# JingInAI/Quantize

Hardware: AMD Instinct MI355X
Metric: quant-conv2d images/sec at batch 256 (ResNet-50, W8A8) (higher is better)
Workload: dtype int8

## Files before the change

### quantize_amd/csrc/qe_conv_plan.hip

```cpp
#include "qe_conv_plan.hpp"

#include <algorithm>
#include <cstdlib>

namespace qe {

static int knob(const char *name, int dflt)
{
    const char *e = env_get(name);
    return e ? atoi(e) : dflt;
}

static size_t align_up(size_t v, size_t a) { return (v + a - 1) / a * a; }

static const int kNiw[3][3] = {{7, 4, 2}, {4, 2, 1}, {2, 1, 0}};
static const int kWN[3] = {1, 2, 4};

struct PlanFront {
    MfmaPlan p;
    int max_tiles = 0;
    bool ok = false;
};

static PlanFront plan_front(const qe_conv_shape *sh)
// ... 227 lines not shown
    if (p.family == MfmaFamily::None) p = plan_flat_s2(f, sh, w_bits);
    if (p.family == MfmaFamily::None) p = plan_flatg(f, sh, w_bits);
    if (p.family == MfmaFamily::None) {
        if (stem_shape(sh)) p = plan_stem(f, sh);
        else {
            p = plan_sm2(f, sh);
            if (p.family == MfmaFamily::None) p = plan_halo(f, sh);
        }
    }
    if (p.family == MfmaFamily::None) return f.p;
    return plan_tables(p, sh);
}

static qe_conv_shape dense_shape(const qe_conv_shape *sh)
{
    qe_conv_shape d = *sh;
    d.H = (sh->H - 1) / sh->stride + 1;
    d.W = (sh->W - 1) / sh->stride + 1;
    d.stride = 1;
    return d;
}

static MfmaPlan make_plan(const qe_conv_shape *sh, int x_bits, int w_bits)
{
    const bool expand = x_bits < 8;
    const int sub_env = knob("QE_SUBSAMPLE", -1);
    const int p_out = ((sh->H - 1) / std::max(1, (int)sh->stride) + 1) * ((sh->W - 1) / std::max(1, (int)sh->stride) + 1);
    const bool sub_x4 = x_bits == 4 && sh->stride == 2 && (sh->W % 2) == 0 && ((int64_t)sh->H * sh->W % 2) == 0 &&
                        knob("QE_SUB_X4", 1) != 0;
    const bool sub = sh->KH == 1 && sh->KW == 1 && sh->stride > 1 && sh->padding == 0 && sub_env != 0 &&
                     (sub_env > 0 || p_out <= 256 || sub_x4);
    const qe_conv_shape ds = dense_shape(sh);
    if (x_bits == 4 && !sub && knob("QE_X4", 1) != 0) {
        const PlanFront f = plan_front(sh);
        MfmaPlan q = f.ok ? plan_flat(f, sh, w_bits, true) : f.p;
        if (q.family == MfmaFamily::FlatX4) {
            q = plan_tables(q, sh);
            q.prep_total = q.total;
            return q;
        }
    }
    MfmaPlan p = make_plan8(sub ? &ds : sh, w_bits);
    p.prep_total = p.total;
    if (p.family != MfmaFamily::None && sub) {
        p.sub = true;
        p.sub_x4 = sub_x4;
        p.sub_off = align_up(p.total, 256);
        p.total = p.sub_off + align_up((size_t)ds.N * ds.IC * ds.H * ds.W, 256);
    } else if (sub) {
        p = make_plan8(sh, w_bits);
        p.prep_total = p.total;
    }
    if (p.family != MfmaFamily::None && expand) {
        p.expand = true;
        p.xe_off = align_up(p.total, 256);
        p.total = p.xe_off + align_up((size_t)sh->N * sh->IC * sh->H * sh->W, 256);
    }
    return p;
}

MfmaPlan plan_prepared(const qe_conv_shape *sh, int x_bits, int w_bits)
{
    qe_conv_shape s1 = *sh;
    const int64_t img = (int64_t)sh->IC * sh->H * sh->W;
    s1.N = img >= 64 ? 1 : (int)((64 + img - 1) / img);
    return make_plan(&s1, x_bits, w_bits);
}

uint64_t prepared_layout(const MfmaPlan &p, const qe_conv_shape *sh)
{
    if (p.family == MfmaFamily::None || p.prep_total == 0) return 0;
    uint64_t h = 1469598103934665603ull;
    auto mix = [&](uint64_t v) { h = (h ^ v) * 1099511628211ull; };
    mix(p.family == MfmaFamily::Stem ? 1 : 0); mix((uint64_t)p.OCP); mix((uint64_t)p.NG); mix((uint64_t)p.KK); mix((uint64_t)sh->KH); mix((uint64_t)sh->KW);
    mix((uint64_t)sh->IC); mix((uint64_t)sh->OC); mix((uint64_t)p.prep_total); mix((uint64_t)p.ep_off); mix((uint64_t)p.ws_off);
    return h | 1ull;
}

struct PwrFit {
    int tw = 0, ks = 0, groups = 1;
    bool s2 = false;
};

static bool pwr_plan(const qe_conv_shape *sh, const qe_qparam *x, const qe_qparam *w, uintptr_t xa, PwrFit *pl)
{
    const int mode = knob("QE_PWR", 2);
    if (mode == 0) return false;
    if (sh->KH != 1 || sh->KW != 1 || sh->padding != 0 || (sh->stride != 1 && sh->stride != 2)) return false;
    if (x->n_bits != 8 || w->n_bits != 8 || x->n_param != 1) return false;
    if (sh->IC != 64 && sh->IC != 128 && sh->IC != 256) return false;
    if (sh->OC % 32 != 0 || sh->OC < 128 || sh->N < 1) return false;
    const bool s2 = sh->stride == 2;
    if (s2 && ((sh->H & 1) || (sh->W & 7) || sh->W > 64 || knob("QE_PWR_S2", 1) == 0)) return false;
    const int OH = s2 ? sh->H / 2 : sh->H, OW = s2 ? sh->W / 2 : sh->W;
    const int64_t P = (int64_t)OH * OW;
    const int tw = (P % 224 == 0) ? 224 : ((P % 196 == 0) ? 196 : 0);
    if (tw == 0) return false;
    if (s2 && (tw % OW != 0 || tw / OW > 8)) return false;
    if (mode == 1 && !s2 && P != tw) return false;
    if ((int64_t)sh->N * sh->IC * sh->H * sh->W < 16 || (int64_t)sh->OC * P >= (1ll << 29) || (int64_t)sh->IC * sh->H * sh->W >= (1ll << 31)) return false;
    if ((reinterpret_cast<uintptr_t>(w->data) & 15) != 0 || (xa & (s2 ? 7 : 3)) != 0) return false;
    if ((reinterpret_cast<uintptr_t>(w->scale) & 3) != 0) return false;
    const int ks = sh->IC / 32;
    const int waves = ks == 8 ? 8 : 4;
    if (sh->OC < 64 * waves) return false;
    const int strips = sh->OC / 32;
    const int g = knob("QE_PWR_GROUPS", 0);
    pl->tw = tw; pl->ks = ks; pl->groups = (g >= 1 && strips % g == 0) ? g : 1; pl->s2 = s2;
    return true;
}

static int pwr7_plan(const qe_conv_shape *sh, const qe_qparam *x, const qe_qparam *w, uintptr_t xa, int *groups)
{
    if (knob("QE_PWR", 2) == 0 || knob("QE_PWR7", 1) == 0) return 0;
    if (sh->KH != 1 || sh->KW != 1 || sh->stride != 1 || sh->padding != 0 || sh->H * sh->W != 49) return 0;
    if (x->n_bits != 8 || w->n_bits != 8 || x->n_param != 1) return 0;
    if (sh->IC != 128 && sh->IC != 256 && sh->IC != 512) return 0;
    const int gi = sh->IC == 512 ? 2 : 4;
    if (sh->OC % 32 != 0 || sh->OC < 512 || sh->N < gi || sh->N % gi != 0) return 0;
    if ((int64_t)sh->N * sh->IC * 49 >= (1ll << 31) || (int64_t)sh->OC * 49 >= (1ll << 29)) return 0;
    if ((reinterpret_cast<uintptr_t>(w->data) & 15) != 0 || (xa & 15) != 0) return 0;
    const int tiles = sh->N / gi, strips = sh->OC / 32;
    int g = 1;
    while (tiles * g < kNumCU && strips % (2 * g) == 0 && strips / (2 * g) >= 8) g *= 2;
    const int ge = knob("QE_PWR_GROUPS", 0);
    *groups = (ge >= 1 && strips % ge == 0) ? ge : g;
    return gi;
}

static bool flatd_plan(const qe_conv_shape *sh, const qe_qparam *x, const qe_qparam *w, uintptr_t xa)
{
    if (sh->KH != 1 || sh->KW != 1 || sh->stride != 1 || sh->padding != 0) return false;
    if (x->n_bits != 8 || w->n_bits != 8 || x->n_param != 1) return false;
    if (sh->IC % FD_CK != 0 || sh->IC < 2 * FD_CK || sh->OC < 1 || sh->N < 1) return false;
    const int64_t P = (int64_t)sh->H * sh->W;
    if ((int64_t)sh->N * sh->IC * P < 16 || (int64_t)sh->OC * P >= (1ll << 29) || (int64_t)sh->IC * P >= (1ll << 31)) return false;
    if ((reinterpret_cast<uintptr_t>(w->data) & 15) != 0) return false;
    return P == 49 && sh->OC % 4 == 0 && (xa & 15) == 0;
}

static bool plan_rq_patch(const MfmaPlan &m, const ConvRequest &r, int split)
{
    if (m.GI != 1 || (m.OH * m.OW) % 4 != 0 || (m.TH * m.OW) % 4 != 0) return false;
    if ((r.rq_out & 3) != 0 || knob("QE_RQ_PATCH", 1) == 0) return false;
    return mfma_instance(m, r.sh->KW, split, true, true) != nullptr;
}

static void plan_mfma_launch(ConvPlan &p, const ConvRequest &r, bool rq)
{
    const MfmaPlan &m = p.m;
    const qe_conv_shape *sh = &p.run;
    p.tiles_h = (m.OH + m.TH - 1) / m.TH;
    p.n_pix_tiles = ((sh->N + m.GI - 1) / m.GI) * p.tiles_h;
    p.n_oc_tiles = m.OCP / m.MT;
    const bool flatg = m.family == MfmaFamily::Flatg;
    const bool flat = mfma_is_flat(m.family);
    if (flatg) {
        p.tiles_h = 1;
        p.n_pix_tiles = (sh->N + m.GI - 1) / m.GI;
    } else if (flat) {
        p.tiles_h = m.IHT;
        p.n_pix_tiles = sh->N * p.tiles_h;
    }
    p.blocks = tile_grid(p.n_pix_tiles, p.tiles_h, p.n_oc_tiles, true, p.chunk);
    auto clipped_lo = [](int pad, int stride, int O) { return std::min(O, (pad + stride - 1) / stride); };
    auto clipped_hi = [](int I, int pad, int K, int stride, int O) {
        const int full_last = (I + pad - K) >= 0 ? (I + pad - K) / stride : -1;
        return std::max(0, std::min(O, O - 1 - full_last));
    };
    p.n_top = clipped_lo(sh->padding, sh->stride, m.OH);
    p.n_bot = clipped_hi(sh->H, sh->padding, sh->KH, sh->stride, m.OH);
    p.n_lft = clipped_lo(sh->padding, sh->stride, m.OW);
    p.n_rgt = clipped_hi(sh->W, sh->padding, sh->KW, sh->stride, m.OW);

    if (flat || flatg) {
        p.lds = m.lds;
        if (rq) {
            p.ptab_off = (int)align_up(m.lds, 16);
            p.lds = p.ptab_off + (flatg ? (size_t)m.GI * m.MT * sh->H * sh->W : (size_t)m.MT * 32 * m.ni);
        }
        return;
    }
    const int units = m.GI * m.IHT * ((sh->W + 3) / 4);
    p.split = units <= 64 ? 4 : (units <= 128 ? 2 : 1);
    p.rq_patch = rq && plan_rq_patch(m, r, p.split);
    const size_t stage_bytes = p.rq_patch ? std::max(m.lds, (size_t)32 * 1024) : m.lds;
    size_t lds_e = stage_bytes;
    const size_t tab = (size_t)m.MT * (sh->KH + 1) * (sh->KW + 1) * sizeof(int);
    const size_t off = align_up(stage_bytes, 16);
    if (off + tab <= (size_t)(m.family == MfmaFamily::Sm2 ? MF_MAX_LDS_SM2 : MF_MAX_LDS)) { p.ptab_off = (int)off; lds_e = off + tab; }
    const int ncls = (1 + p.n_top + p.n_bot) * (1 + p.n_lft + p.n_rgt);
    p.ctab = p.ptab_off != 0 && p.n_top + p.n_bot < m.OH && p.n_lft + p.n_rgt < m.OW && ncls <= (sh->KH + 1) * (sh->KW + 1) &&
             knob("QE_CTAB", 1) != 0;
    p.lds = (m.family == MfmaFamily::Ws && !p.ctab) ? m.lds : lds_e;
}

ConvPlan plan_conv(const ConvRequest &r)
{
    ConvPlan p;
    const qe_conv_shape *sh = r.sh;
    p.OH = (sh->H + 2 * sh->padding - sh->KH) / sh->stride + 1;
    p.OW = (sh->W + 2 * sh->padding - sh->KW) / sh->stride + 1;
    if (p.OH > 0 && p.OW > 0) p.y_bytes = align_up((size_t)sh->N * sh->OC * p.OH * p.OW * sizeof(float), 256);
    p.m = make_plan(sh, r.x->n_bits, r.w->n_bits);
    const MfmaPlan &m = p.m;
    if (r.x->n_param != 1 || m.family == MfmaFamily::None) return p;
    p.run = m.sub ? dense_shape(sh) : *sh;
    const qe_conv_shape *rs = &p.run;

    qe_qparam xr = *r.x;
    uintptr_t xa = reinterpret_cast<uintptr_t>(r.x->data);
    if (m.sub_x4 || m.expand) { xr.n_bits = 8; xr.sign = 1; }
    if (m.sub || m.expand) xa = 0;
    if (m.sub_x4) {
        p.pre = PrePass::SubX4;
        p.pre_blocks = ((int64_t)sh->N * sh->IC * rs->H * ((rs->W + 7) / 8) + 255) / 256;
    } else if (m.sub) {
        const int64_t n_planes = (int64_t)sh->N * sh->IC;
        const int nq = (rs->W + 7) / 8;
        int log_nq = 0;
        while ((1 << log_nq) < nq) ++log_nq;
        const int units2 = rs->H << log_nq;
        if (sh->stride == 2 && (sh->H % 2) == 0 && (1 << log_nq) == nq && 16 * nq <= 2 * sh->W && units2 <= 256 &&
            knob("QE_SUB2", 1) != 0) {
            int log_up = 3;
            while ((1 << log_up) < units2) ++log_up;
            p.pre = PrePass::Sub2;
            p.sub2_log_nq = log_nq;
            p.sub2_log_up = log_up;
            const int ppb = (256 >> log_up) * 4;
            p.pre_blocks = (n_planes + ppb - 1) / ppb;
        } else {
            const bool wide = sh->stride == 2 && (sh->W % 4) == 0 && sh->W >= 16;
            const int units = rs->H * ((rs->W + (wide ? 7 : 3)) / (wide ? 8 : 4));
            const int ppb = units >= 1024 ? 1 : 1024 / units;
            p.pre = wide ? PrePass::SubWide : PrePass::SubNarrow;
            p.pre_blocks = (n_planes + ppb - 1) / ppb;
        }
    }
    if (p.pre_blocks > 0x7fffffffLL) return p;

    PwrFit pf;
    int g7 = 1;
    if (r.residual) {
        if (r.rq_bits != 0 && (r.rq_bits != 8 || r.rq_n_param != 1)) return p;
        if (m.sub || m.expand || rs->stride != 1) return p;
        if (pwr_plan(rs, &xr, r.w, xa, &pf)) p.route = ConvRoute::Pwr;
        else if (rs->IC == 512 && (p.pwr7_gi = pwr7_plan(rs, &xr, r.w, xa, &g7)) != 0) p.route = ConvRoute::Pwr7;
        else return p;
        p.fused = true;
    } else {
        const bool rq = r.rq_bits > 0;
        if (rq) {
            if (r.rq_bits != 8 || r.rq_n_param != 1) return p;
            if (m.family == MfmaFamily::Flatg || mfma_is_flat(m.family)) {
                const size_t patch = m.family == MfmaFamily::Flatg ? (size_t)m.GI * m.MT * rs->H * rs->W : (size_t)m.MT * 32 * m.ni;
                if (align_up(m.lds, 16) + patch > (size_t)MF_MAX_LDS) return p;
            }
            p.fused = true;
        }
        const bool pwr_ok = rq ? (r.rq_out & 15) == 0 && knob("QE_PWR_RQ", 1) != 0 : true;
        const bool fd_ok = flatd_plan(rs, &xr, r.w, xa) && knob("QE_FLATD", 1) != 0 &&
                           (!rq || (rs->OC % 32 == 0 && (r.rq_out & 15) == 0 && knob("QE_FLATD_RQ", 1) != 0));
        if (pwr_ok && pwr_plan(rs, &xr, r.w, xa, &pf)) p.route = ConvRoute::Pwr;
        else if (pwr_ok && (rq || (r.out & 15) == 0) && (p.pwr7_gi = pwr7_plan(rs, &xr, r.w, xa, &g7)) != 0) p.route = ConvRoute::Pwr7;
        else if (fd_ok) p.route = ConvRoute::Flatd;
        else p.route = ConvRoute::Mfma;
    }

    if (p.route == ConvRoute::Pwr) {
        p.pwr_tw = pf.tw; p.pwr_ks = pf.ks; p.pwr_groups = pf.groups; p.pwr_s2 = pf.s2;
        const int64_t P = pf.s2 ? (int64_t)(rs->H / 2) * (rs->W / 2) : (int64_t)rs->H * rs->W;
        p.tiles_h = (int)(P / pf.tw);
        p.n_pix_tiles = rs->N * p.tiles_h;
        p.blocks = tile_grid(p.n_pix_tiles, p.tiles_h, pf.groups, true, p.chunk);
    } else if (p.route == ConvRoute::Pwr7) {
        p.pwr_groups = g7;
        p.tiles_h = 1;
        p.n_pix_tiles = rs->N / p.pwr7_gi;
        p.blocks = tile_grid(p.n_pix_tiles, 1, g7, false, p.chunk);
    } else if (p.route == ConvRoute::Flatd) {
        const char *e8 = env_get("QE_FLATD8");
        p.fd_w8 = e8 ? atoi(e8) != 0 && rs->OC > 128 : rs->OC >= 1024;
        const int MT = p.fd_w8 ? 256 : 128;
        p.n_oc_tiles = (rs->OC + MT - 1) / MT;
        p.tiles_h = 1;
        p.n_pix_tiles = (rs->N + 3) / 4;
        p.blocks = tile_grid(p.n_pix_tiles, p.tiles_h, p.n_oc_tiles, true, p.chunk);
    } else {
        plan_mfma_launch(p, r, p.fused);
    }
    if (p.blocks > 0x7fffffffLL) { p.route = ConvRoute::Generic; p.fused = false; }
    return p;
}

}
```

### quantize_amd/csrc/qe_conv_plan.hpp

```cpp
#pragma once
#include "qe_conv_common.hpp"

namespace qe {

constexpr int FD_CK = 64;

enum class MfmaFamily {
    None,
    Halo,
    Ws,
    Sm2,
    Stem,
    Flat,
    FlatS2,
    FlatX4,
    Flatg
};

inline bool mfma_is_flat(MfmaFamily f) { return f == MfmaFamily::Flat || f == MfmaFamily::FlatS2 || f == MfmaFamily::FlatX4; }

struct MfmaPlan {
    MfmaFamily family = MfmaFamily::None;
    int cfg = 0;
    int MT = 0, OCP = 0, NCH = 0, NG = 0, KK = 0, OH = 0, OW = 0;
    int TH = 0, ni = 0, niw = 0, IHT = 0, IWP = 0, ROWMUL = 1, COLMUL = 1;
    int GI = 1, NS = 1;
    bool wraw = false;
    bool expand = false;
    size_t xe_off = 0;
    bool sub = false;
    bool sub_x4 = false;
    size_t sub_off = 0;
    size_t lds = 0;
    size_t wt_bytes = 0, ep_off = 0, ws_off = 0, total = 0;
    size_t prep_total = 0;
};

enum class ConvRoute { Generic, Pwr, Pwr7, Flatd, Mfma };
enum class PrePass { None, SubX4, Sub2, SubWide, SubNarrow };

struct ConvRequest {
    const qe_conv_shape *sh;
    const qe_qparam *x, *w;
    uintptr_t out = 0;
    uintptr_t rq_out = 0;
    int rq_bits = 0;
    int rq_n_param = 1;
    bool residual = false;
};

struct ConvPlan {
    ConvRoute route = ConvRoute::Generic;
    bool fused = false;
    int OH = 0, OW = 0;
    size_t y_bytes = 0;
    MfmaPlan m;
    qe_conv_shape run{};

    PrePass pre = PrePass::None;
    int64_t pre_blocks = 0;
    int sub2_log_up = 0, sub2_log_nq = 0;

    int64_t blocks = 0;
    int chunk = 1, n_pix_tiles = 0, n_oc_tiles = 0, tiles_h = 0;
    size_t lds = 0;

    int pwr_tw = 0, pwr_ks = 0, pwr_groups = 1, pwr7_gi = 0;
    bool pwr_s2 = false;
    bool fd_w8 = false;
    bool rq_patch = false;
    bool ctab = false;
    int ptab_off = 0;
    int n_top = 0, n_bot = 0, n_lft = 0, n_rgt = 0;
    int split = 1;
};

ConvPlan plan_conv(const ConvRequest &rq);
MfmaPlan plan_prepared(const qe_conv_shape *sh, int x_bits, int w_bits);
uint64_t prepared_layout(const MfmaPlan &p, const qe_conv_shape *sh);

MfmaLaunch mfma_instance(const MfmaPlan &m, int KW, int split, bool rq, bool patch);
inline int mfma_kkt(int KK, int KW) { return KK == 1 ? 1 : ((KK == 9 && KW == 3) ? 9 : 0); }

int launch_conv_mfma(const ConvPlan &p, const qe_qparam *x, const qe_qparam *w, const float *bias, const qe_conv_shape *sh,
                     float *out, void *workspace, size_t workspace_bytes, const void *prepared, size_t prepared_bytes,
                     bool use_prepared, hipStream_t s, const RequantHost *rq, const float *res);
int prepare_conv_tables(const MfmaPlan &p, const qe_qparam *w, const float *bias, const qe_conv_shape *sh, void *prepared,
                        size_t prepared_bytes, hipStream_t s);
int launch_pwr(const ConvPlan &p, const qe_qparam *x, const qe_qparam *w, const float *bias, float *out, hipStream_t s,
               const RequantHost *rq, const float *res);
int launch_flatd(const ConvPlan &p, const qe_qparam *x, const qe_qparam *w, const float *bias, float *out, hipStream_t s,
                 const RequantHost *rq);

enum class F32Kernel {
    Stem4x1x7, Stem2x2x4, Stem2x2x7,
    M4x1x4, M4x1x4S2, M4x1x7, M4x1x7S2, M2x2x2, M2x2x2S2, M2x2x4, M2x2x4S2
};

struct F32Plan {
    bool ok = false;
    F32Kernel kernel = F32Kernel::M4x1x7;
    bool stem = false;
    int OCP = 0, NG = 0, KK = 0, OH = 0, OW = 0;
    int TH = 0, GI = 1, IHT = 0, IWP = 0, ROWMUL = 1, COLMUL = 1;
    int64_t blocks = 0;
    int chunk = 1, n_pix_tiles = 0, n_oc_tiles = 0, tiles_h = 0;
    size_t lds = 0;
    size_t ep_off = 0, total = 0;
};

F32Plan plan_conv_f32(const qe_conv_shape *sh);
int prepare_conv_f32(const F32Plan &p, const qe_qparam *w, const float *bias, const qe_conv_shape *sh, void *prepared,
                     size_t prepared_bytes, hipStream_t s);
int launch_conv_f32(const F32Plan &p, const float *x, const qe_conv_shape *sh, const void *prepared, size_t prepared_bytes,
                    float *out, hipStream_t s);

}
```

### quantize_amd/csrc/qe_conv_pwr.hip

```cpp
#include "qe_conv_common.hpp"
#include "qe_conv_plan.hpp"

#include <utility>

namespace qe {

struct PwrArgs {
    const uint8_t *x;
    const uint8_t *w;
    const float *x_scale, *x_zero, *w_scale, *w_zero, *bias;
    int x_sign, w_sign, w_per_tensor;
    float *out;
    int N, IC, OC, P;
    int tiles_per_image, n_pix_tiles, chunk;
    int n_groups;
    int strips_per_group;
    unsigned long long *dbg;
    int W_in, PIN, OW;
    RqArgs rq;
    const float *res;
};

template <bool RQ, int NB> struct ResBlock {
    float4 v[NB];
    uint32_t pk[RQ ? NB : 1];
    int64_t e;
};
template <int NB>
__device__ __forceinline__ void res_load(const PwrArgs &a, int64_t e, const uint32_t (&off)[NB], float4 (&id)[NB])
{
#pragma unroll
    for (int k = 0; k < NB; ++k) id[k] = *reinterpret_cast<const float4 *>(a.res + e + off[k]);
}
template <bool RQ, int NB>
__device__ __forceinline__ void res_flush(const PwrArgs &a, const ResBlock<RQ, NB> &b, const uint32_t (&off)[NB])
{
    if (a.out != nullptr) {
#pragma unroll
        for (int k = 0; k < NB; ++k) *reinterpret_cast<float4 *>(a.out + b.e + off[k]) = b.v[k];
    }
    if constexpr (RQ) {
#pragma unroll
        for (int k = 0; k < NB; ++k) *reinterpret_cast<uint32_t *>(a.rq.out + b.e + off[k]) = b.pk[k];
    }
}
template <bool RQ>
__device__ __forceinline__ void res_make(const RqConst &rqc, float4 y, float4 id, float4 &out, uint32_t &pk, bool &bad)
{
    float v[4] = {y.x + id.x, y.y + id.y, y.z + id.z, y.w + id.w};
#pragma unroll
    for (int j = 0; j < 4; ++j) v[j] = (v[j] > 0.0f || v[j] != v[j]) ? v[j] : 0.0f;
    out = make_float4(v[0], v[1], v[2], v[3]);
    if constexpr (RQ) {
        pk = 0;
#pragma unroll
        for (int j = 0; j < 4; ++j) {
            bool b = false;
            const float r = rq_value(rqc, v[j], b);
            bad |= b;
            pk = __builtin_amdgcn_cvt_pk_u8_f32(r, j, pk);
        }
    }
}

template <int NT, int WAVES, int KS, int TW> struct PwrGeom {
    static constexpr int THREADS = 64 * WAVES;
    static constexpr int IC = 32 * KS;
    static constexpr int RS = 32 * NT;
    static constexpr int NTP = 32 * NT;
    static constexpr int XBYTES = IC * RS;
    static constexpr int XINSTR = XBYTES / 1024;
    static constexpr int PXW = (XINSTR + WAVES - 1) / WAVES;
    static constexpr int TAB = WAVES * 4 * 32 * 4;
    static constexpr int PATCH = 8 * TW * 4;
    static constexpr int PPR = TW / 4;
    static constexpr int NRB = (8 * PPR + 63) / 64;
    static constexpr int PPRB = (TW + 15) / 16;
    static constexpr int NRQ = (32 * PPRB + 63) / 64;
    static constexpr int LDS = XBYTES + TAB + WAVES * PATCH;
};

template <int NT, int WAVES, int KS, int TW, bool S2 = false, bool RQ = false, bool RES = false>
__global__ __launch_bounds__(64 * WAVES, 2) void conv_pwr_kernel(const PwrArgs a)
{
    using G = PwrGeom<NT, WAVES, KS, TW>;
    static_assert(!(S2 && RES), "the residual epilogue has stride-1 instances only");
    constexpr bool RQT = RQ && !RES;
    static_assert(TW % 4 == 0 && TW <= 32 * NT && TW > 32 * (NT - 1), "tile width");
    constexpr int RS = G::RS, PXW = G::PXW;
    static_assert((NT & 1) == 1, "row stride must be an odd multiple of 32 B");
    extern __shared__ __attribute__((aligned(16))) uint8_t smem[];

    const int tid = threadIdx.x, lane = tid & 63;
    const int wave = __builtin_amdgcn_readfirstlane(tid >> 6);
    const int col = lane & 31, h = lane >> 5;
    const int P = a.P;
#ifdef QE_STAMP
    unsigned long long st[8] = {0, 0, 0, 0, 0, 0, 0, 0};
    unsigned long long tprev = qe_stamp();
    const unsigned long long tstart = tprev;
#endif

    int pt, og;
    {
        const int bid = blockIdx.x;
        const int idx = bid >> 3;
        const int j = idx / a.n_groups;
        og = idx - j * a.n_groups;
        const int c = j / a.chunk;
        pt = (c * 8 + (bid & 7)) * a.chunk + (j - c * a.chunk);
    }
    if (pt >= a.n_pix_tiles) return;
    const int n0 = pt / a.tiles_per_image;
    const int p0 = (pt - n0 * a.tiles_per_image) * TW;

    uint8_t *Xs = smem;
    float *tab = reinterpret_cast<float *>(smem + G::XBYTES) + wave * 128;
    float *patch = reinterpret_cast<float *>(smem + G::XBYTES + G::TAB) + wave * (8 * TW);

    const int strip0 = og * a.strips_per_group + wave;
    const int n_my = (a.strips_per_group - wave + WAVES - 1) / WAVES;
    v4i wf[KS];
    float c_sw, c_zw, c_bi;
    auto load_w = [&](int strip) __attribute__((always_inline)) {
        const int oc = strip * 32 + col;
        const float *psw = a.w_scale + (a.w_per_tensor ? 0 : oc);
        const float *pzw = a.w_zero + (a.w_per_tensor ? 0 : oc);
        const float *pbi = a.bias ? a.bias + oc : psw;
        const uint8_t *wl = a.w + (int64_t)oc * G::IC + 16 * h;
        asm volatile("global_load_dword %0, %3, off\n\tglobal_load_dword %1, %4, off\n\tglobal_load_dword %2, %5, off"
                     : "=&v"(c_sw), "=&v"(c_zw), "=&v"(c_bi) : "v"(psw), "v"(pzw), "v"(pbi) : "memory");
#define QE_PWR_LW(K, OFF) if constexpr (KS > K) asm volatile("global_load_dwordx4 %0, %1, off offset:" #OFF : "=v"(wf[K]) : "v"(wl) : "memory")
        QE_PWR_LW(0, 0); QE_PWR_LW(1, 32); QE_PWR_LW(2, 64); QE_PWR_LW(3, 96);
        QE_PWR_LW(4, 128); QE_PWR_LW(5, 160); QE_PWR_LW(6, 192); QE_PWR_LW(7, 224);
#undef QE_PWR_LW
    };
    auto wait_w = [&](auto n_tag) __attribute__((always_inline)) {
        constexpr int N = decltype(n_tag)::value;
        if constexpr (KS == 2) asm volatile("s_waitcnt vmcnt(%5)" : "+v"(c_sw), "+v"(c_zw), "+v"(c_bi), "+v"(wf[0]), "+v"(wf[1]) : "i"(N) : "memory");
        else if constexpr (KS == 4) asm volatile("s_waitcnt vmcnt(%7)" : "+v"(c_sw), "+v"(c_zw), "+v"(c_bi), "+v"(wf[0]), "+v"(wf[1]), "+v"(wf[2]), "+v"(wf[3]) : "i"(N) : "memory");
        else asm volatile("s_waitcnt vmcnt(%11)" : "+v"(c_sw), "+v"(c_zw), "+v"(c_bi), "+v"(wf[0]), "+v"(wf[1]), "+v"(wf[2]), "+v"(wf[3]), "+v"(wf[4]), "+v"(wf[5]), "+v"(wf[6]), "+v"(wf[7]) : "i"(N) : "memory");
        if (!a.bias) c_bi = 0.0f;
    };
    if (n_my > 0) load_w(strip0);

    const int n_xi = (G::XINSTR % WAVES == 0 || wave < G::XINSTR % WAVES) ? PXW : PXW - 1;
    int fix_i = -1;
    uint32_t tail_word = 0;
    if constexpr (S2) {
        constexpr int THREADS = 64 * WAVES;
        constexpr int MAXP = 8;
        const int RT = TW / a.OW;
        const int NU = G::IC * RT;
        const int np = a.W_in >> 3;
        const int r0 = p0 / a.OW;
        const uint8_t *xin = a.x + (int64_t)n0 * G::IC * a.PIN;
        constexpr int UPT = (G::IC * 8 + THREADS - 1) / THREADS;
#pragma unroll
        for (int i0 = 0; i0 < UPT; i0 += 2) {
            uint2 d[2][MAXP];
            int cc[2], rr[2];
            bool live[2];
#pragma unroll
            for (int q = 0; q < 2; ++q) {
                const int u = tid + THREADS * (i0 + q);
                live[q] = (i0 + q) < UPT && u < NU;
                const int uc = live[q] ? u : 0;
                cc[q] = uc / RT; rr[q] = uc - cc[q] * RT;
                const uint8_t *row = xin + (int64_t)cc[q] * a.PIN + (int64_t)(2 * (r0 + rr[q])) * a.W_in;
#pragma unroll
                for (int j = 0; j < MAXP; ++j) {
                    const int jc = j < np ? j : np - 1;
                    __builtin_memcpy(&d[q][j], row + 8 * jc, 8);
                }
            }
#pragma unroll
            for (int q = 0; q < 2; ++q) {
                uint32_t *dst = reinterpret_cast<uint32_t *>(Xs + cc[q] * RS + rr[q] * a.OW);
#pragma unroll
                for (int j = 0; j < MAXP; ++j)
                    if (live[q] && j < np) dst[j] = __builtin_amdgcn_perm(d[q][j].y, d[q][j].x, 0x06040200u) ^ 0x80808080u;
            }
        }
    } else {
    const int64_t x_total = (int64_t)a.N * G::IC * P;
    const int64_t x_last16 = x_total - 16;
    tail_word = *reinterpret_cast<const uint32_t *>(a.x + x_total - 4);
#pragma unroll
    for (int i = 0; i < PXW; ++i) {
        const int e = 64 * (wave + WAVES * i) + lane;
        const int c = e / (RS / 16);
        const int j = e - c * (RS / 16);
        int64_t src = ((int64_t)n0 * G::IC + c) * P + p0 + 16 * j;
        bool skip = false;
        if (src > x_last16) {
            if (src < x_total && i < n_xi) { skip = true; fix_i = i; }
            else src = x_last16;
        }
        if (i < n_xi && !skip)
            __builtin_amdgcn_global_load_lds((const __attribute__((address_space(1))) void *)(a.x + src),
                                             (__attribute__((address_space(3))) void *)(Xs + 1024 * (wave + WAVES * i)), 16, 0, 0);
    }

    }

    constexpr int NRB = G::NRB;
    uint32_t rb_off[NRB];
#pragma unroll
    for (int k = 0; k < NRB; ++k) {
        const int f = 64 * k + lane;
        const int row = f / G::PPR, pc = f - row * G::PPR;
        rb_off[k] = f < 8 * G::PPR ? (uint32_t)row * (uint32_t)P + 4u * (uint32_t)pc : 0u;
    }

    uint32_t rs_off[RES ? NRB : 1], rs_lds[RES ? NRB : 1];
    if constexpr (RES) {
#pragma unroll
        for (int k = 0; k < NRB; ++k) {
            const int f = (64 * k + lane) < 8 * G::PPR ? 64 * k + lane : 8 * G::PPR - 1;
            const int row = f / G::PPR, pc = f - row * G::PPR;
            rs_off[k] = (uint32_t)row * (uint32_t)P + 4u * (uint32_t)pc;
            rs_lds[k] = 4u * (uint32_t)f;
        }
    }

    uint32_t rq_lds[RQT ? G::NRQ : 1], rq_glb[RQT ? G::NRQ : 1];
    bool rq_live[RQT ? G::NRQ : 1];
    if constexpr (RQT) {
#pragma unroll
        for (int k = 0; k < G::NRQ; ++k) {
            const int f = 64 * k + lane;
            if (P == TW) {
// ... 474 lines not shown
                    if (64 * k + lane < 98) *reinterpret_cast<uint4 *>(dst + 16 * (64 * k + lane)) = d4;
                }
            }
            return;
        }
#pragma unroll
        for (int gi = 0; gi < GI; ++gi) {
#pragma unroll
            for (int gq = 0; gq < 4; ++gq) {
                const float4 al = *reinterpret_cast<const float4 *>(tab + 8 * gq + 4 * h);
                const float4 cs = *reinterpret_cast<const float4 *>(tab + 32 + 8 * gq + 4 * h);
                const float4 bi = *reinterpret_cast<const float4 *>(tab + 64 + 8 * gq + 4 * h);
                const float alv[4] = {al.x, al.y, al.z, al.w}, csv[4] = {cs.x, cs.y, cs.z, cs.w};
                const float biv[4] = {bi.x, bi.y, bi.z, bi.w};
                float zwv[4] = {0.0f, 0.0f, 0.0f, 0.0f};
                if (need_sx) {
                    const float4 zw = *reinterpret_cast<const float4 *>(tab + 96 + 8 * gq + 4 * h);
                    zwv[0] = zw.x; zwv[1] = zw.y; zwv[2] = zw.z; zwv[3] = zw.w;
                }
#pragma unroll
                for (int tt = 0; tt < 2; ++tt) {
                    const int t = 2 * gi + tt;
                    const int px = 32 * tt + col;
#pragma unroll
                    for (int j = 0; j < 4; ++j) {
                        float f = (float)acc[t][4 * gq + j] + csv[j];
                        if (need_sx) f = fmaf(-zwv[j], sxv[t], f);
                        const float v = fmaf(alv[j], f, biv[j]);
                        if (tt == 0 || px < P) patch[(8 * gq + 4 * h + j) * P + px] = v;
                    }
                }
            }
            if constexpr (RES) {
                const int64_t e_g = ((int64_t)(n0 + gi) * a.OC + oc0) * P;
                float4 id[NRB];
                res_load(a, e_g, rs_off, id);
                if (gi > 0) res_flush(a, pend, rs_off);
#pragma unroll
                for (int k = 0; k < NRB; ++k)
                    res_make<RQ>(rqc, *reinterpret_cast<const float4 *>(patch + rs_off[k]), id[k], pend.v[k], pend.pk[RQ ? k : 0], bad);
                pend.e = e_g;
                continue;
            }
            float *dst = a.out + ((int64_t)(n0 + gi) * a.OC + oc0) * P;
#pragma unroll
            for (int k = 0; k < NRB; ++k) {
                const float4 o4 = *reinterpret_cast<const float4 *>(patch + 4 * (64 * k + lane));
                if (64 * k + 64 <= 392 || 64 * k + lane < 392) *reinterpret_cast<float4 *>(dst + 4 * (64 * k + lane)) = o4;
            }
        }
        if constexpr (RES) res_flush(a, pend, rs_off);
    };

    bool sx_cur = __builtin_amdgcn_ballot_w64((c_zw - zw_shift) != 0.0f) != 0ull;
    if (sx_cur) mma_strip(std::true_type{}); else mma_strip(std::false_type{});
    for (int s = 0; s + 1 < n_my; ++s) {
        const float e_sw = c_sw, e_zw = c_zw, e_bi = c_bi;
        load_w(strip0 + (s + 1) * WAVES);
        epilogue(strip0 + s * WAVES, e_sw, e_zw, e_bi, sx_cur);
        QE_PWR7_WAIT(RES ? 63 : (RQ ? 2 : NRB) * GI);
        sx_cur = __builtin_amdgcn_ballot_w64((c_zw - zw_shift) != 0.0f) != 0ull;
        if (sx_cur) mma_strip(std::true_type{}); else mma_strip(std::false_type{});
    }
    epilogue(strip0 + (n_my - 1) * WAVES, c_sw, c_zw, c_bi, sx_cur);
    if constexpr (RQ) rq_report(a.rq, bad);
#undef QE_PWR7_WAIT
}

template <int KSV, int GIV, bool RQV, bool RESV>
static void launch_pwr7_k(const PwrArgs &a, int64_t blocks, hipStream_t s)
{
    constexpr size_t lds = Pwr7Geom<KSV, GIV>::LDS;
    launch_instance<&conv_pwr7_kernel<KSV, GIV, RQV, RESV>>((unsigned)blocks, 512, lds, lds, s, a);
}
template <int KSV, int GIV, bool RESV>
static void launch_pwr7_rq(const PwrArgs &a, bool rq, int64_t blocks, hipStream_t s)
{
    if (rq) launch_pwr7_k<KSV, GIV, true, RESV>(a, blocks, s); else launch_pwr7_k<KSV, GIV, false, RESV>(a, blocks, s);
}
template <int WV, int KSV, int TWV, bool S2V, bool RQV>
static void launch_pwr_k(const PwrArgs &a, int64_t blocks, hipStream_t s)
{
    constexpr size_t lds = PwrGeom<7, WV, KSV, TWV>::LDS;
    launch_instance<&conv_pwr_kernel<7, WV, KSV, TWV, S2V, RQV>>((unsigned)blocks, 64 * WV, lds, lds, s, a);
}
template <int WV, int KSV, int TWV, bool RQV>
static void launch_pwr_res(const PwrArgs &a, int64_t blocks, hipStream_t s)
{
    constexpr size_t lds = PwrGeom<7, WV, KSV, TWV>::LDS;
    launch_instance<&conv_pwr_kernel<7, WV, KSV, TWV, false, RQV, true>>((unsigned)blocks, 64 * WV, lds, lds, s, a);
}
template <int WV, int KSV, int TWV>
static void launch_pwr_tile(const PwrArgs &a, bool s2, bool rq, bool res, int64_t blocks, hipStream_t s)
{
    if (res) { if (rq) launch_pwr_res<WV, KSV, TWV, true>(a, blocks, s); else launch_pwr_res<WV, KSV, TWV, false>(a, blocks, s); }
    else if (s2) { if (rq) launch_pwr_k<WV, KSV, TWV, true, true>(a, blocks, s); else launch_pwr_k<WV, KSV, TWV, true, false>(a, blocks, s); }
    else { if (rq) launch_pwr_k<WV, KSV, TWV, false, true>(a, blocks, s); else launch_pwr_k<WV, KSV, TWV, false, false>(a, blocks, s); }
}

static void launch_pwr7(const ConvPlan &p, const qe_qparam *x, const qe_qparam *w, const float *bias, float *out, hipStream_t s,
                        const RequantHost *rq, const float *res)
{
    const qe_conv_shape *sh = &p.run;
    PwrArgs a;
    a.res = res;
    a.rq = make_rq_args(rq);
    a.W_in = 7; a.PIN = 49; a.OW = 7;
    a.x = static_cast<const uint8_t *>(x->data); a.w = static_cast<const uint8_t *>(w->data);
    a.x_scale = x->scale; a.x_zero = x->zero; a.w_scale = w->scale; a.w_zero = w->zero; a.bias = bias;
    a.x_sign = x->sign; a.w_sign = w->sign; a.w_per_tensor = (w->n_param == 1);
    a.out = out; a.N = sh->N; a.IC = sh->IC; a.OC = sh->OC; a.P = 49;
    a.tiles_per_image = 1;
    a.n_pix_tiles = p.n_pix_tiles;
    a.n_groups = p.pwr_groups;
    a.strips_per_group = sh->OC / 32 / p.pwr_groups;
    a.dbg = g_mfma_dbg;
    a.chunk = p.chunk;
    const int64_t blocks = p.blocks;
    if (res != nullptr) launch_pwr7_rq<16, 2, true>(a, rq != nullptr, blocks, s);
    else if (sh->IC == 512) launch_pwr7_rq<16, 2, false>(a, rq != nullptr, blocks, s);
    else if (sh->IC == 256) launch_pwr7_rq<8, 4, false>(a, rq != nullptr, blocks, s);
    else launch_pwr7_rq<4, 4, false>(a, rq != nullptr, blocks, s);
}

int launch_pwr(const ConvPlan &p, const qe_qparam *x, const qe_qparam *w, const float *bias, float *out, hipStream_t s,
               const RequantHost *rq, const float *res)
{
    if (p.route == ConvRoute::Pwr7) {
        launch_pwr7(p, x, w, bias, out, s, rq, res);
        QE_LAUNCH_CHECK();
        return QE_OK;
    }
    const qe_conv_shape *sh = &p.run;
    PwrArgs a;
    a.res = res;
    a.rq = make_rq_args(rq);
    a.x = static_cast<const uint8_t *>(x->data); a.w = static_cast<const uint8_t *>(w->data);
    a.x_scale = x->scale; a.x_zero = x->zero; a.w_scale = w->scale; a.w_zero = w->zero; a.bias = bias;
    a.x_sign = x->sign; a.w_sign = w->sign; a.w_per_tensor = (w->n_param == 1);
    a.out = out; a.N = sh->N; a.IC = sh->IC; a.OC = sh->OC;
    a.W_in = sh->W; a.PIN = sh->H * sh->W;
    a.OW = p.pwr_s2 ? sh->W / 2 : sh->W;
    a.P = p.pwr_s2 ? (sh->H / 2) * (sh->W / 2) : sh->H * sh->W;
    a.tiles_per_image = p.tiles_h;
    a.n_pix_tiles = p.n_pix_tiles;
    a.n_groups = p.pwr_groups;
    a.strips_per_group = sh->OC / 32 / p.pwr_groups;
    a.dbg = g_mfma_dbg;
    a.chunk = p.chunk;
    const int64_t blocks = p.blocks;
    const bool rqv = rq != nullptr, resv = res != nullptr;
    if (p.pwr_tw == 224) {
        if (p.pwr_ks == 2) launch_pwr_tile<4, 2, 224>(a, p.pwr_s2, rqv, resv, blocks, s);
        else if (p.pwr_ks == 4) launch_pwr_tile<4, 4, 224>(a, p.pwr_s2, rqv, resv, blocks, s);
        else launch_pwr_tile<8, 8, 224>(a, p.pwr_s2, rqv, resv, blocks, s);
    } else {
        if (p.pwr_ks == 2) launch_pwr_tile<4, 2, 196>(a, p.pwr_s2, rqv, resv, blocks, s);
        else if (p.pwr_ks == 4) launch_pwr_tile<4, 4, 196>(a, p.pwr_s2, rqv, resv, blocks, s);
        else launch_pwr_tile<8, 8, 196>(a, p.pwr_s2, rqv, resv, blocks, s);
    }
    QE_LAUNCH_CHECK();
    return QE_OK;
}

}
```

Measured before the change: 62350.

## Route stride-2 1x1 IC=512 convs directly through the pointwise kernel

Adds a KS=16 (IC=512) stride-2 instance of the pointwise conv kernel with a dedicated input-staging path that subsamples rows of a 28-wide map while loading into LDS. The planner can now send strided 1x1 convs that previously needed a separate subsample pre-pass straight to this kernel, removing the extra pass and its intermediate buffer. Launch dispatch is rebuilt as a table of instances, and launch bounds drop to one block per CU for KS>=16, which trades occupancy for registers.

```diff
diff --git a/quantize_amd/csrc/qe_conv_plan.hip b/quantize_amd/csrc/qe_conv_plan.hip
--- a/quantize_amd/csrc/qe_conv_plan.hip
+++ b/quantize_amd/csrc/qe_conv_plan.hip
@@ -333,27 +333,28 @@
     bool s2 = false;
 };
 
-static bool pwr_plan(const qe_conv_shape *sh, const qe_qparam *x, const qe_qparam *w, uintptr_t xa, PwrFit *pl)
+static bool pwr_plan(const qe_conv_shape *sh, const qe_qparam *x, const qe_qparam *w, uintptr_t xa, bool rq, bool res, PwrFit *pl)
 {
     const int mode = knob("QE_PWR", 2);
     if (mode == 0) return false;
     if (sh->KH != 1 || sh->KW != 1 || sh->padding != 0 || (sh->stride != 1 && sh->stride != 2)) return false;
     if (x->n_bits != 8 || w->n_bits != 8 || x->n_param != 1) return false;
-    if (sh->IC != 64 && sh->IC != 128 && sh->IC != 256) return false;
+    if (sh->IC != 64 && sh->IC != 128 && sh->IC != 256 && sh->IC != 512) return false;
     if (sh->OC % 32 != 0 || sh->OC < 128 || sh->N < 1) return false;
     const bool s2 = sh->stride == 2;
-    if (s2 && ((sh->H & 1) || (sh->W & 7) || sh->W > 64 || knob("QE_PWR_S2", 1) == 0)) return false;
+    if (s2 && ((sh->H & 1) || (sh->IC == 512 ? sh->W != 28 : (sh->W & 7) != 0) || sh->W > 64 || knob("QE_PWR_S2", 1) == 0)) return false;
     const int OH = s2 ? sh->H / 2 : sh->H, OW = s2 ? sh->W / 2 : sh->W;
     const int64_t P = (int64_t)OH * OW;
     const int tw = (P % 224 == 0) ? 224 : ((P % 196 == 0) ? 196 : 0);
     if (tw == 0) return false;
-    if (s2 && (tw % OW != 0 || tw / OW > 8)) return false;
+    if (s2 && (tw % OW != 0 || tw / OW > (sh->IC == 512 ? 14 : 8))) return false;
     if (mode == 1 && !s2 && P != tw) return false;
     if ((int64_t)sh->N * sh->IC * sh->H * sh->W < 16 || (int64_t)sh->OC * P >= (1ll << 29) || (int64_t)sh->IC * sh->H * sh->W >= (1ll << 31)) return false;
     if ((reinterpret_cast<uintptr_t>(w->data) & 15) != 0 || (xa & (s2 ? 7 : 3)) != 0) return false;
     if ((reinterpret_cast<uintptr_t>(w->scale) & 3) != 0) return false;
     const int ks = sh->IC / 32;
-    const int waves = ks == 8 ? 8 : 4;
+    const int waves = pwr_instance_waves(ks, tw, s2, rq, res);
+    if (waves == 0) return false;
     if (sh->OC < 64 * waves) return false;
     const int strips = sh->OC / 32;
     const int g = knob("QE_PWR_GROUPS", 0);
@@ -456,6 +457,16 @@
     p.m = make_plan(sh, r.x->n_bits, r.w->n_bits);
     const MfmaPlan &m = p.m;
     if (r.x->n_param != 1 || m.family == MfmaFamily::None) return p;
+    PwrFit pf;
+    bool pwr_direct = false;
+    {
+        const bool pwr_ok0 = r.rq_bits > 0 ? (r.rq_out & 15) == 0 && knob("QE_PWR_RQ", 1) != 0 : true;
+        if (m.sub && !m.sub_x4 && !m.expand && !r.residual && knob("QE_SUBSAMPLE", -1) <= 0 && pwr_ok0 &&
+            pwr_plan(sh, r.x, r.w, reinterpret_cast<uintptr_t>(r.x->data), r.rq_bits > 0, false, &pf)) {
+            p.m.sub = false;
+            pwr_direct = true;
+        }
+    }
     p.run = m.sub ? dense_shape(sh) : *sh;
     const qe_conv_shape *rs = &p.run;
 
@@ -491,12 +502,11 @@
     }
     if (p.pre_blocks > 0x7fffffffLL) return p;
 
-    PwrFit pf;
     int g7 = 1;
     if (r.residual) {
         if (r.rq_bits != 0 && (r.rq_bits != 8 || r.rq_n_param != 1)) return p;
         if (m.sub || m.expand || rs->stride != 1) return p;
-        if (pwr_plan(rs, &xr, r.w, xa, &pf)) p.route = ConvRoute::Pwr;
+        if (pwr_plan(rs, &xr, r.w, xa, r.rq_bits != 0, true, &pf)) p.route = ConvRoute::Pwr;
         else if (rs->IC == 512 && (p.pwr7_gi = pwr7_plan(rs, &xr, r.w, xa, &g7)) != 0) p.route = ConvRoute::Pwr7;
         else return p;
         p.fused = true;
@@ -513,7 +523,7 @@
         const bool pwr_ok = rq ? (r.rq_out & 15) == 0 && knob("QE_PWR_RQ", 1) != 0 : true;
         const bool fd_ok = flatd_plan(rs, &xr, r.w, xa) && knob("QE_FLATD", 1) != 0 &&
                            (!rq || (rs->OC % 32 == 0 && (r.rq_out & 15) == 0 && knob("QE_FLATD_RQ", 1) != 0));
-        if (pwr_ok && pwr_plan(rs, &xr, r.w, xa, &pf)) p.route = ConvRoute::Pwr;
+        if (pwr_direct || (pwr_ok && pwr_plan(rs, &xr, r.w, xa, rq, false, &pf))) p.route = ConvRoute::Pwr;
         else if (pwr_ok && (rq || (r.out & 15) == 0) && (p.pwr7_gi = pwr7_plan(rs, &xr, r.w, xa, &g7)) != 0) p.route = ConvRoute::Pwr7;
         else if (fd_ok) p.route = ConvRoute::Flatd;
         else p.route = ConvRoute::Mfma;
diff --git a/quantize_amd/csrc/qe_conv_plan.hpp b/quantize_amd/csrc/qe_conv_plan.hpp
--- a/quantize_amd/csrc/qe_conv_plan.hpp
+++ b/quantize_amd/csrc/qe_conv_plan.hpp
@@ -89,6 +89,7 @@
                         size_t prepared_bytes, hipStream_t s);
 int launch_pwr(const ConvPlan &p, const qe_qparam *x, const qe_qparam *w, const float *bias, float *out, hipStream_t s,
                const RequantHost *rq, const float *res);
+int pwr_instance_waves(int ks, int tw, bool s2, bool rq, bool res);
 int launch_flatd(const ConvPlan &p, const qe_qparam *x, const qe_qparam *w, const float *bias, float *out, hipStream_t s,
                  const RequantHost *rq);
 
diff --git a/quantize_amd/csrc/qe_conv_pwr.hip b/quantize_amd/csrc/qe_conv_pwr.hip
--- a/quantize_amd/csrc/qe_conv_pwr.hip
+++ b/quantize_amd/csrc/qe_conv_pwr.hip
@@ -81,7 +81,7 @@
 };
 
 template <int NT, int WAVES, int KS, int TW, bool S2 = false, bool RQ = false, bool RES = false>
-__global__ __launch_bounds__(64 * WAVES, 2) void conv_pwr_kernel(const PwrArgs a)
+__global__ __launch_bounds__(64 * WAVES, KS >= 16 ? 1 : 2) void conv_pwr_kernel(const PwrArgs a)
 {
     using G = PwrGeom<NT, WAVES, KS, TW>;
     static_assert(!(S2 && RES), "the residual epilogue has stride-1 instances only");
@@ -133,13 +133,17 @@
 #define QE_PWR_LW(K, OFF) if constexpr (KS > K) asm volatile("global_load_dwordx4 %0, %1, off offset:" #OFF : "=v"(wf[K]) : "v"(wl) : "memory")
         QE_PWR_LW(0, 0); QE_PWR_LW(1, 32); QE_PWR_LW(2, 64); QE_PWR_LW(3, 96);
         QE_PWR_LW(4, 128); QE_PWR_LW(5, 160); QE_PWR_LW(6, 192); QE_PWR_LW(7, 224);
+        QE_PWR_LW(8, 256); QE_PWR_LW(9, 288); QE_PWR_LW(10, 320); QE_PWR_LW(11, 352);
+        QE_PWR_LW(12, 384); QE_PWR_LW(13, 416); QE_PWR_LW(14, 448); QE_PWR_LW(15, 480);
 #undef QE_PWR_LW
     };
     auto wait_w = [&](auto n_tag) __attribute__((always_inline)) {
         constexpr int N = decltype(n_tag)::value;
         if constexpr (KS == 2) asm volatile("s_waitcnt vmcnt(%5)" : "+v"(c_sw), "+v"(c_zw), "+v"(c_bi), "+v"(wf[0]), "+v"(wf[1]) : "i"(N) : "memory");
         else if constexpr (KS == 4) asm volatile("s_waitcnt vmcnt(%7)" : "+v"(c_sw), "+v"(c_zw), "+v"(c_bi), "+v"(wf[0]), "+v"(wf[1]), "+v"(wf[2]), "+v"(wf[3]) : "i"(N) : "memory");
-        else asm volatile("s_waitcnt vmcnt(%11)" : "+v"(c_sw), "+v"(c_zw), "+v"(c_bi), "+v"(wf[0]), "+v"(wf[1]), "+v"(wf[2]), "+v"(wf[3]), "+v"(wf[4]), "+v"(wf[5]), "+v"(wf[6]), "+v"(wf[7]) : "i"(N) : "memory");
+        else if constexpr (KS == 8) asm volatile("s_waitcnt vmcnt(%11)" : "+v"(c_sw), "+v"(c_zw), "+v"(c_bi), "+v"(wf[0]), "+v"(wf[1]), "+v"(wf[2]), "+v"(wf[3]), "+v"(wf[KS - 4]), "+v"(wf[KS - 3]), "+v"(wf[KS - 2]), "+v"(wf[KS - 1]) : "i"(N) : "memory");
+        else asm volatile("s_waitcnt vmcnt(%19)" : "+v"(c_sw), "+v"(c_zw), "+v"(c_bi), "+v"(wf[0]), "+v"(wf[1]), "+v"(wf[2]), "+v"(wf[3]), "+v"(wf[4]), "+v"(wf[5]), "+v"(wf[6]), "+v"(wf[7]),
+                          "+v"(wf[KS - 8]), "+v"(wf[KS - 7]), "+v"(wf[KS - 6]), "+v"(wf[KS - 5]), "+v"(wf[KS - 4]), "+v"(wf[KS - 3]), "+v"(wf[KS - 2]), "+v"(wf[KS - 1]) : "i"(N) : "memory");
         if (!a.bias) c_bi = 0.0f;
     };
     if (n_my > 0) load_w(strip0);
@@ -147,7 +151,39 @@
     const int n_xi = (G::XINSTR % WAVES == 0 || wave < G::XINSTR % WAVES) ? PXW : PXW - 1;
     int fix_i = -1;
     uint32_t tail_word = 0;
-    if constexpr (S2) {
+    if constexpr (S2 && KS == 16) {
+        constexpr int THREADS = 64 * WAVES, RT = 14, NU = G::IC * RT, UPT = NU / THREADS, UIF = 14;
+        static_assert(TW == 196 && NU % THREADS == 0 && UPT % UIF == 0, "whole rounds of units");
+        const uint8_t *xin = a.x + (int64_t)n0 * G::IC * a.PIN + (int64_t)(2 * (p0 / RT)) * 28;
+#pragma unroll
+        for (int i0 = 0; i0 < UPT; i0 += UIF) {
+            uint2 d[UIF][3];
+            uint32_t e[UIF], lo[UIF];
+#pragma unroll
+            for (int q = 0; q < UIF; ++q) {
+                const int u = tid + THREADS * (i0 + q);
+                const int c = u / RT, r = u - c * RT;
+                const uint8_t *row = xin + (int64_t)c * a.PIN + 56 * r;
+                lo[q] = (uint32_t)(c * RS + r * RT);
+#pragma unroll
+                for (int j = 0; j < 3; ++j) __builtin_memcpy(&d[q][j], row + 8 * j, 8);
+                __builtin_memcpy(&e[q], row + 24, 4);
+            }
+#pragma unroll
+            for (int q = 0; q < UIF; ++q) {
+                const uint32_t w0 = __builtin_amdgcn_perm(d[q][0].y, d[q][0].x, 0x06040200u) ^ 0x80808080u;
+                const uint32_t w1 = __builtin_amdgcn_perm(d[q][1].y, d[q][1].x, 0x06040200u) ^ 0x80808080u;
+                const uint32_t w2 = __builtin_amdgcn_perm(d[q][2].y, d[q][2].x, 0x06040200u) ^ 0x80808080u;
+                const uint32_t w3 = __builtin_amdgcn_perm(e[q], e[q], 0x06040200u) ^ 0x80808080u;
+                const bool odd = (lo[q] & 2u) != 0;
+                const uint32_t b32 = lo[q] + (odd ? 2u : 0u), b16 = lo[q] + (odd ? 0u : 12u);
+                *reinterpret_cast<uint32_t *>(Xs + b32) = odd ? __builtin_amdgcn_alignbit(w1, w0, 16) : w0;
+                *reinterpret_cast<uint32_t *>(Xs + b32 + 4) = odd ? __builtin_amdgcn_alignbit(w2, w1, 16) : w1;
+                *reinterpret_cast<uint32_t *>(Xs + b32 + 8) = odd ? __builtin_amdgcn_alignbit(w3, w2, 16) : w2;
+                *reinterpret_cast<uint16_t *>(Xs + b16) = (uint16_t)(odd ? w0 : w3);
+            }
+        }
+    } else if constexpr (S2) {
         constexpr int THREADS = 64 * WAVES;
         constexpr int MAXP = 8;
         const int RT = TW / a.OW;
@@ -788,20 +824,47 @@
 static void launch_pwr_k(const PwrArgs &a, int64_t blocks, hipStream_t s)
 {
     constexpr size_t lds = PwrGeom<7, WV, KSV, TWV>::LDS;
+    static_assert(lds <= 160 * 1024, "the CU's LDS");
     launch_instance<&conv_pwr_kernel<7, WV, KSV, TWV, S2V, RQV>>((unsigned)blocks, 64 * WV, lds, lds, s, a);
 }
 template <int WV, int KSV, int TWV, bool RQV>
 static void launch_pwr_res(const PwrArgs &a, int64_t blocks, hipStream_t s)
 {
     constexpr size_t lds = PwrGeom<7, WV, KSV, TWV>::LDS;
+    static_assert(lds <= 160 * 1024, "the CU's LDS");
     launch_instance<&conv_pwr_kernel<7, WV, KSV, TWV, false, RQV, true>>((unsigned)blocks, 64 * WV, lds, lds, s, a);
 }
-template <int WV, int KSV, int TWV>
-static void launch_pwr_tile(const PwrArgs &a, bool s2, bool rq, bool res, int64_t blocks, hipStream_t s)
-{
-    if (res) { if (rq) launch_pwr_res<WV, KSV, TWV, true>(a, blocks, s); else launch_pwr_res<WV, KSV, TWV, false>(a, blocks, s); }
-    else if (s2) { if (rq) launch_pwr_k<WV, KSV, TWV, true, true>(a, blocks, s); else launch_pwr_k<WV, KSV, TWV, true, false>(a, blocks, s); }
-    else { if (rq) launch_pwr_k<WV, KSV, TWV, false, true>(a, blocks, s); else launch_pwr_k<WV, KSV, TWV, false, false>(a, blocks, s); }
+
+struct PwrInstance {
+    int waves, ks, tw;
+    bool s2, rq, res;
+    void (*launch)(const PwrArgs &a, int64_t blocks, hipStream_t s);
+};
+#define QE_PWR_FORMS(WV, KS, TW)                                                                                          \
+    {WV, KS, TW, false, false, false, &launch_pwr_k<WV, KS, TW, false, false>},                                           \
+    {WV, KS, TW, false, true, false, &launch_pwr_k<WV, KS, TW, false, true>},                                             \
+    {WV, KS, TW, true, false, false, &launch_pwr_k<WV, KS, TW, true, false>},                                             \
+    {WV, KS, TW, true, true, false, &launch_pwr_k<WV, KS, TW, true, true>},                                               \
+    {WV, KS, TW, false, false, true, &launch_pwr_res<WV, KS, TW, false>},                                                 \
+    {WV, KS, TW, false, true, true, &launch_pwr_res<WV, KS, TW, true>}
+static const PwrInstance kPwrInstances[] = {
+    QE_PWR_FORMS(4, 2, 224), QE_PWR_FORMS(4, 4, 224), QE_PWR_FORMS(8, 8, 224),
+    QE_PWR_FORMS(4, 2, 196), QE_PWR_FORMS(4, 4, 196), QE_PWR_FORMS(8, 8, 196),
+    {4, 16, 196, true, false, false, &launch_pwr_k<4, 16, 196, true, false>},
+};
+#undef QE_PWR_FORMS
+
+static const PwrInstance *pwr_instance(int ks, int tw, bool s2, bool rq, bool res)
+{
+    for (const PwrInstance &i : kPwrInstances)
+        if (i.ks == ks && i.tw == tw && i.s2 == s2 && i.rq == rq && i.res == res) return &i;
+    return nullptr;
+}
+
+int pwr_instance_waves(int ks, int tw, bool s2, bool rq, bool res)
+{
+    const PwrInstance *i = pwr_instance(ks, tw, s2, rq, res);
+    return i ? i->waves : 0;
 }
 
 static void launch_pwr7(const ConvPlan &p, const qe_qparam *x, const qe_qparam *w, const float *bias, float *out, hipStream_t s,
@@ -854,17 +917,9 @@
     a.strips_per_group = sh->OC / 32 / p.pwr_groups;
     a.dbg = g_mfma_dbg;
     a.chunk = p.chunk;
-    const int64_t blocks = p.blocks;
-    const bool rqv = rq != nullptr, resv = res != nullptr;
-    if (p.pwr_tw == 224) {
-        if (p.pwr_ks == 2) launch_pwr_tile<4, 2, 224>(a, p.pwr_s2, rqv, resv, blocks, s);
-        else if (p.pwr_ks == 4) launch_pwr_tile<4, 4, 224>(a, p.pwr_s2, rqv, resv, blocks, s);
-        else launch_pwr_tile<8, 8, 224>(a, p.pwr_s2, rqv, resv, blocks, s);
-    } else {
-        if (p.pwr_ks == 2) launch_pwr_tile<4, 2, 196>(a, p.pwr_s2, rqv, resv, blocks, s);
-        else if (p.pwr_ks == 4) launch_pwr_tile<4, 4, 196>(a, p.pwr_s2, rqv, resv, blocks, s);
-        else launch_pwr_tile<8, 8, 196>(a, p.pwr_s2, rqv, resv, blocks, s);
-    }
+    const PwrInstance *inst = pwr_instance(p.pwr_ks, p.pwr_tw, p.pwr_s2, rq != nullptr, res != nullptr);
+    if (inst == nullptr) return QE_ERR_UNSUPPORTED;
+    inst->launch(a, p.blocks, s);
     QE_LAUNCH_CHECK();
     return QE_OK;
 }
```

New measurement: 62680, median of 6. About the same (+0.5%).
